# manyeyes/K2TransducerAsr

Hardware: AMD Instinct MI355X
Metric: RTFx (audio-sec/wall-sec) offline Zipformer greedy (higher is better)
Workload: dtype f32

## Files before the change

k2transducerasr_amd/csrc/attn.hip:

```cpp
#include "kernels.h"

namespace k2hip {

typedef float f32x16 __attribute__((ext_vector_type(16)));

namespace {

constexpr int PH = 4;
constexpr int R = 32;

template <int NG>
__global__ __launch_bounds__(512, 4) void k_attn_scores_softmax(const float* __restrict__ qkp, int ld,
                                                             const float* __restrict__ pp, float* __restrict__ aw, int B,
                                                             int T, int Tp, int H, int lds_stride, int koff0, int poff0) {
    constexpr int QH = 8 * NG;
    extern __shared__ __attribute__((aligned(16))) float S[];
    const int tid = threadIdx.x, lane = tid & 63, wave = tid >> 6;
    const int li = lane & 31, lh = lane >> 5;
    const int i0 = blockIdx.x * R, b = blockIdx.y, h = blockIdx.z;
    const float* base = qkp + (long long)b * T * ld;
    const int qoff = h * QH, koff = koff0 + h * QH, poff = poff0 + h * PH;
    const int ppld = H * PH;

    float4 fq[NG];
    {
        int row = i0 + li;
#pragma unroll
        for (int g = 0; g < NG; g++) {
            fq[g] = make_float4(0.f, 0.f, 0.f, 0.f);
            if (row < T) fq[g] = *reinterpret_cast<const float4*>(base + (long long)row * ld + qoff + 8 * g + 4 * lh);
        }
    }
    const int njt = (T + 31) / 32;
    float4 fkn[NG];
    auto load_keys = [&](int jt) {
        if (jt >= njt) return;
        const int j = min(jt * 32 + li, T - 1);
#pragma unroll
        for (int g = 0; g < NG; g++) fkn[g] = *reinterpret_cast<const float4*>(base + (long long)j * ld + koff + 8 * g + 4 * lh);
    };
    load_keys(wave);
    float4* PW = reinterpret_cast<float4*>(S + R * lds_stride);
    const int nlo = T - 1 - min(i0 + R - 1, T - 1), nwin = (2 * T - 2 - i0) - nlo + 1;
    for (int wdx = tid; wdx < nwin; wdx += 512) PW[wdx] = *reinterpret_cast<const float4*>(pp + (long long)(nlo + wdx) * ppld + h * PH);
    float4* PR = PW + (T + R);
    if (tid < R) PR[tid] = i0 + tid < T ? *reinterpret_cast<const float4*>(base + (long long)(i0 + tid) * ld + poff) : make_float4(0.f, 0.f, 0.f, 0.f);
    __syncthreads();

    for (int jt = wave; jt < njt; jt += 8) {
        int j = jt * 32 + li;
        float4 fk[NG];
#pragma unroll
        for (int g = 0; g < NG; g++) fk[g] = fkn[g];
        load_keys(jt + 8);
        f32x16 acc;
#pragma unroll
        for (int r = 0; r < 16; r++) acc[r] = 0.f;
#pragma unroll
        for (int g = 0; g < NG; g++) {
            acc = __builtin_amdgcn_mfma_f32_32x32x2f32(fq[g].x, fk[g].x, acc, 0, 0, 0);
            acc = __builtin_amdgcn_mfma_f32_32x32x2f32(fq[g].y, fk[g].y, acc, 0, 0, 0);
            acc = __builtin_amdgcn_mfma_f32_32x32x2f32(fq[g].z, fk[g].z, acc, 0, 0, 0);
            acc = __builtin_amdgcn_mfma_f32_32x32x2f32(fq[g].w, fk[g].w, acc, 0, 0, 0);
        }
        if (j < T) {
#pragma unroll
            for (int r0 = 0; r0 < 16; r0 += 8) {
                float4 e[8];
#pragma unroll
                for (int r = 0; r < 8; r++) {
                    const int rl = ((r0 + r) & 3) + 8 * ((r0 + r) >> 2) + 4 * lh;
                    e[r] = PW[T - 1 - min(i0 + rl, T - 1) + j - nlo];
                }
#pragma unroll
                for (int r = 0; r < 8; r++) {
                    const int rl = ((r0 + r) & 3) + 8 * ((r0 + r) >> 2) + 4 * lh;
                    const float4 pq = PR[rl];
                    S[rl * lds_stride + j] = acc[r0 + r] + (pq.x * e[r].x + pq.y * e[r].y + pq.z * e[r].z + pq.w * e[r].w);
                }
            }
        }
    }
    __syncthreads();

    float* out = aw + (((long long)h * B + b) * T) * Tp;
    if (Tp <= 1024) {
        float4 v[4][4];
        const int nk = (Tp + 255) >> 8;
#pragma unroll
        for (int rr = 0; rr < 4; rr++) {
            const float* srow = S + (wave * 4 + rr) * lds_stride;
#pragma unroll
            for (int k = 0; k < 4; k++) {
                const int j4 = lane * 4 + 256 * k;
                v[rr][k] = make_float4(-INFINITY, -INFINITY, -INFINITY, -INFINITY);
                if (k < nk && j4 < T) {
                    const float4 t = *reinterpret_cast<const float4*>(srow + j4);
                    v[rr][k].x = t.x;
                    if (j4 + 1 < T) v[rr][k].y = t.y;
                    if (j4 + 2 < T) v[rr][k].z = t.z;
                    if (j4 + 3 < T) v[rr][k].w = t.w;
                }
            }
        }
#pragma unroll
        for (int rr = 0; rr < 4; rr++) {
            const int i = i0 + wave * 4 + rr;
            if (i >= T) break;
            float mx = -INFINITY;
#pragma unroll
            for (int k = 0; k < 4; k++)
                if (k < nk) mx = fmaxf(fmaxf(fmaxf(mx, v[rr][k].x), fmaxf(v[rr][k].y, v[rr][k].z)), v[rr][k].w);
            mx = wave_max_dpp(mx);
            float sum = 0.f;
#pragma unroll
            for (int k = 0; k < 4; k++) {
                if (k >= nk) break;
                v[rr][k].x = __expf(v[rr][k].x - mx); v[rr][k].y = __expf(v[rr][k].y - mx);
                v[rr][k].z = __expf(v[rr][k].z - mx); v[rr][k].w = __expf(v[rr][k].w - mx);
                sum += (v[rr][k].x + v[rr][k].y) + (v[rr][k].z + v[rr][k].w);
            }
#pragma unroll
            for (int o = 32; o > 0; o >>= 1) sum += __shfl_xor(sum, o);
            const float inv = 1.0f / sum;
            float* orow = out + (long long)i * Tp;
#pragma unroll
            for (int k = 0; k < 4; k++) {
                const int j4 = lane * 4 + 256 * k;
                if (k < nk && j4 < Tp) *reinterpret_cast<float4*>(orow + j4) = make_float4(v[rr][k].x * inv, v[rr][k].y * inv, v[rr][k].z * inv, v[rr][k].w * inv);
            }
        }
        return;
    }
// ... 406 lines not shown
    }
    const int ct0 = blockIdx.z * tiles_per_z, ct1 = min(D >> 4, ct0 + tiles_per_z);
    const float* ar = cs_ + n * CS + 4 * kq;
    for (int ct = ct0 + wave; ct < ct1; ct += NWV) {
        const int col = ct * 16 + n;
        const float* wr = wout + (long long)col * Hc + 4 * kq;
        const float bvv = bias[col];
        float xr[4];
#pragma unroll
        for (int e = 0; e < 4; e++) {
            const int i = 4 * kq + e;
            xr[e] = i < T ? x[((long long)b * T + i) * D + col] : 0.f;
        }
        f32x4 acc0 = {0.f, 0.f, 0.f, 0.f}, acc1 = {0.f, 0.f, 0.f, 0.f};
        for (int c0 = 0; c0 < Hc; c0 += 64) {
            float4 w4[4], a4[4];
#pragma unroll
            for (int g = 0; g < 4; g++) {
                const bool ok = c0 + 16 * g + 4 * kq < Hc;
                w4[g] = ok ? *reinterpret_cast<const float4*>(wr + c0 + 16 * g) : make_float4(0.f, 0.f, 0.f, 0.f);
                a4[g] = ok ? *reinterpret_cast<const float4*>(ar + c0 + 16 * g) : make_float4(0.f, 0.f, 0.f, 0.f);
            }
#pragma unroll
            for (int g = 0; g < 4; g++) {
                if (g & 1) {
                    acc1 = __builtin_amdgcn_mfma_f32_16x16x4f32(a4[g].x, w4[g].x, acc1, 0, 0, 0);
                    acc1 = __builtin_amdgcn_mfma_f32_16x16x4f32(a4[g].y, w4[g].y, acc1, 0, 0, 0);
                    acc1 = __builtin_amdgcn_mfma_f32_16x16x4f32(a4[g].z, w4[g].z, acc1, 0, 0, 0);
                    acc1 = __builtin_amdgcn_mfma_f32_16x16x4f32(a4[g].w, w4[g].w, acc1, 0, 0, 0);
                } else {
                    acc0 = __builtin_amdgcn_mfma_f32_16x16x4f32(a4[g].x, w4[g].x, acc0, 0, 0, 0);
                    acc0 = __builtin_amdgcn_mfma_f32_16x16x4f32(a4[g].y, w4[g].y, acc0, 0, 0, 0);
                    acc0 = __builtin_amdgcn_mfma_f32_16x16x4f32(a4[g].z, w4[g].z, acc0, 0, 0, 0);
                    acc0 = __builtin_amdgcn_mfma_f32_16x16x4f32(a4[g].w, w4[g].w, acc0, 0, 0, 0);
                }
            }
        }
        float o[4];
#pragma unroll
        for (int e = 0; e < 4; e++) o[e] = acc0[e] + acc1[e] + bvv + xr[e];
        float* xp = x + ((long long)b * T + 4 * kq) * D + col;
#pragma unroll
        for (int e = 0; e < 4; e++)
            if (4 * kq + e < T) xp[(long long)e * D] = o[e];
    }
}

}

template <int NG>
static void attn_scores_launch(const Ctx& ctx, const float* qkp, int ld, const float* pp, float* aw, int B, int T, int Tp, int H, int koff0,
                               int poff0) {
    int lds_stride = Tp + 4;
    size_t lds = sizeof(float) * (R * lds_stride + 4 * (T + R) + 4 * R);
    const bool force_long = tunables().attn_long != 0;
    if (lds > 160 * 1024 || force_long) {
        hipLaunchKernelGGL(k_attn_scores_softmax_long<NG>, dim3(cdiv(T, R), B, H), dim3(256), 0, ctx.stream, qkp, ld, pp, aw, B, T, Tp, H, koff0,
                           poff0);
        K2_HIP(hipGetLastError());
        return;
    }
    static LdsAttrOnce lds_attr;
    lds_attr.ensure(k_attn_scores_softmax<NG>, 160 * 1024);
    dim3 grid(cdiv(T, R), B, H);
    hipLaunchKernelGGL(k_attn_scores_softmax<NG>, grid, dim3(512), lds, ctx.stream, qkp, ld, pp, aw, B, T, Tp, H, lds_stride, koff0, poff0);
    K2_HIP(hipGetLastError());
}

void attn_scores_softmax(const Ctx& ctx, const float* qkp, int ld, const float* pp, float* aw, int B, int T, int Tp, int H, int qh, int koff0,
                         int poff0) {
    K2_REQUIRE(Tp % 4 == 0 && Tp >= T, "attn: Tp=%d must be T=%d rounded up to 4", Tp, T);
    if (koff0 < 0) koff0 = H * qh;
    if (poff0 < 0) poff0 = 2 * H * qh;
    K2_REQUIRE(koff0 % 4 == 0 && poff0 % 4 == 0 && ld % 4 == 0, "attn: operand offsets must be multiples of 4 floats");
    ctx.add_flops(0.0, 2.0 * (qh + PH) * (double)T * T * B * H, 0);
    if (ctx.dry) return;
    switch (qh) {
        case 32: attn_scores_launch<4>(ctx, qkp, ld, pp, aw, B, T, Tp, H, koff0, poff0); break;
        case 24: attn_scores_launch<3>(ctx, qkp, ld, pp, aw, B, T, Tp, H, koff0, poff0); break;
        case 16: attn_scores_launch<2>(ctx, qkp, ld, pp, aw, B, T, Tp, H, koff0, poff0); break;
        default: failf(K2HIP_ERR_UNSUPPORTED, "attention head size %d unsupported (16, 24, 32)", qh);
    }
}

bool attn_av_out(const Ctx& ctx, const float* aw, const float* v, const float* wout, const float* bias, float* x, int B, int T, int KL, int Tp,
                 int H, int vh, int D) {
    const int HV = H * vh, Tk = (KL + 63) & ~63;
    const bool off = tunables().no_fused_av != 0;
    if (off || vh > 16 || HV % 4 != 0 || HV > 128 || D % 16 != 0 || Tp % 4 != 0 || Tp < KL) return false;
    ctx.add_flops(0.0, 2.0 * B * (double)T * HV * (KL + D), 0);
    if (ctx.dry) return true;
    const int strips = cdiv(T, 16) * B, ntile = D / 16;
    int cs = std::max(1, std::min(4, 512 / std::max(1, strips)));
    cs = std::min(cs, ntile);
    const int tiles_per_z = cdiv(ntile, cs);
    cs = cdiv(ntile, tiles_per_z);
    const size_t lds = sizeof(float) * 16 * (HV + 1);
    hipLaunchKernelGGL(k_attn_av_out<false>, dim3(cdiv(T, 16), B, cs), dim3(256), lds, ctx.stream, aw, v, wout, bias, x, B, T, KL, Tp, Tk, H, vh,
                       D, tiles_per_z, RingRef(), nullptr);
    K2_HIP(hipGetLastError());
    return true;
}

bool attn_av_out_ring(const Ctx& ctx, const float* aw, const RingRef& vals, const float* newrows, const float* wout, const float* bias, float* x,
                      int B, int T, int KL, int Tp, int H, int vh, int D) {
    const int HV = H * vh, Tk = (KL + 63) & ~63;
    K2_REQUIRE(vh <= 16 && HV % 4 == 0 && HV <= 128 && D % 16 == 0 && Tp % 4 == 0 && Tp >= KL && T <= 16,
// ... 71 lines not shown
```

k2transducerasr_amd/csrc/elementwise.hip:

```cpp
#include "kernels.h"

namespace k2hip {
namespace {

constexpr float kLogFloor = -23.025850929940457F;

__device__ __forceinline__ float fast_softplus(float z) { return z > 15.f ? z : __logf(1.0f + __expf(z)); }
__device__ __forceinline__ float swoosh_r(float v) { return fast_softplus(v - 1.0f) - 0.08f * v - 0.313261687f; }
__device__ __forceinline__ float fast_tanh(float v) {
    float e = __expf(-2.0f * fabsf(v));
    float t = (1.0f - e) / (1.0f + e);
    return v < 0.f ? -t : t;
}

__device__ __forceinline__ float sigm(float s) { return 1.0f / (1.0f + __expf(-s)); }
__device__ __forceinline__ float dswish(float v) { return v / (1.0f + __expf(1.0f - v)); }

inline int nblocks(long long n, int per) { return (int)((n + per - 1) / per); }

__global__ void k_pad_logfloor(const float* __restrict__ packed, const long long* __restrict__ off,
                               const long long* __restrict__ len, float* __restrict__ out, long long L) {
    int b = blockIdx.y;
    const float* src = packed + off[b];
    long long n = len[b];
    for (long long j = (long long)blockIdx.x * blockDim.x + threadIdx.x; j < L; j += (long long)gridDim.x * blockDim.x) {
        float v = j < n ? src[j] : 0.0f;
        out[(long long)b * L + j] = (v == 0.0f) ? kLogFloor : v;
    }
}
__global__ void k_pad_logfloor_dense(const float* __restrict__ feats, long long n, float* __restrict__ out, long long L) {
    int b = blockIdx.y;
    for (long long j = (long long)blockIdx.x * blockDim.x + threadIdx.x; j < L; j += (long long)gridDim.x * blockDim.x) {
        float v = j < n ? feats[(long long)b * n + j] : 0.0f;
        out[(long long)b * L + j] = (v == 0.0f) ? kLogFloor : v;
    }
}

template <int TPAD, bool DSWISH>
__global__ void k_conv0(const float* __restrict__ x, const float* __restrict__ w, const float* __restrict__ bias,
                        float* __restrict__ y, int B, int T, int F) {
    __shared__ float sw[72], sb[8];
    if (threadIdx.x < 72) sw[threadIdx.x] = w[threadIdx.x];
    if (threadIdx.x < 8) sb[threadIdx.x] = bias[threadIdx.x];
    __syncthreads();
    int T1 = T - 2 + 2 * TPAD;
    long long n = (long long)B * T1 * F;
    long long i = (long long)blockIdx.x * blockDim.x + threadIdx.x;
    if (i >= n) return;
    int f = (int)(i % F);
    long long bt = i / F;
    int t = (int)(bt % T1), b = (int)(bt / T1);
    float xin[3][3];
#pragma unroll
    for (int kt = 0; kt < 3; kt++)
#pragma unroll
        for (int kf = 0; kf < 3; kf++) {
            int ff = f + kf - 1, tt = t + kt - TPAD;
            xin[kt][kf] = (ff >= 0 && ff < F && tt >= 0 && tt < T) ? x[((long long)b * T + tt) * F + ff] : 0.f;
        }
    float o[8];
#pragma unroll
    for (int co = 0; co < 8; co++) {
        float s = sb[co];
#pragma unroll
        for (int kt = 0; kt < 3; kt++)
#pragma unroll
            for (int kf = 0; kf < 3; kf++) s += sw[(co * 3 + kt) * 3 + kf] * xin[kt][kf];
        o[co] = DSWISH ? dswish(s) : swoosh_r(s);
    }
    float4* yo = reinterpret_cast<float4*>(y + i * 8);
    yo[0] = make_float4(o[0], o[1], o[2], o[3]);
// ... 508 lines not shown
    const int q = (int)(i % W4);
    const long long bt = i / W4;
    const int t2 = (int)(bt % Td2), b = (int)(bt / Td2);
    float4 s = make_float4(0.f, 0.f, 0.f, 0.f);
    if (q < D4) {
        const float4 sc = reinterpret_cast<const float4*>(scale)[q];
        for (int k = 0; k < ds2; k++) {
            const int t = t2 * ds2 + k, tt = min(t, T - 1);
            const long long row = (long long)b * T + tt;
            const float4 o = q < Do4 ? reinterpret_cast<const float4*>(orig)[row * Do4 + q] : make_float4(0.f, 0.f, 0.f, 0.f);
            const float4 u = reinterpret_cast<const float4*>(xd)[((long long)b * Td + tt / ds) * D4 + q];
            const float4 v = make_float4(o.x + (u.x - o.x) * sc.x, o.y + (u.y - o.y) * sc.y, o.z + (u.z - o.z) * sc.z, o.w + (u.w - o.w) * sc.w);
            if (t < T) reinterpret_cast<float4*>(y)[row * D4 + q] = v;
            s.x += v.x * wgt[k]; s.y += v.y * wgt[k]; s.z += v.z * wgt[k]; s.w += v.w * wgt[k];
        }
    }
    if (q < D2_4) reinterpret_cast<float4*>(xd2)[((long long)b * Td2 + t2) * D2_4 + q] = s;
}
__global__ void k_convert_channels(const float* __restrict__ x, float* __restrict__ y, long long M, int Din4, int Dout4) {
    long long i = (long long)blockIdx.x * blockDim.x + threadIdx.x;
    if (i >= M * Dout4) return;
    long long m = i / Dout4;
    int q = (int)(i % Dout4);
    reinterpret_cast<float4*>(y)[i] = q < Din4 ? reinterpret_cast<const float4*>(x)[m * Din4 + q] : make_float4(0.f, 0.f, 0.f, 0.f);
}
__global__ void k_copy_cols(const float* __restrict__ x, int ldx, int xc, float* __restrict__ y, int ldy, int yc,
                            long long M, int n4) {
    long long i = (long long)blockIdx.x * blockDim.x + threadIdx.x;
    if (i >= M * n4) return;
    long long m = i / n4;
    int q = (int)(i % n4);
    *reinterpret_cast<float4*>(y + m * ldy + yc + 4 * q) = *reinterpret_cast<const float4*>(x + m * ldx + xc + 4 * q);
}

}

#define LAUNCH(kernel, grid, block, ...)                                        \
    do {                                                                        \
        if (!ctx.dry) {                                                         \
            hipLaunchKernelGGL(kernel, grid, block, 0, ctx.stream, __VA_ARGS__); \
            K2_HIP(hipGetLastError());                                          \
        }                                                                       \
    } while (0)

void pad_logfloor(const Ctx& ctx, const float* packed, const long long* d_off, const long long* d_len, float* out, int B,
                  long long L) {
    dim3 grid(std::min(nblocks(L, 256), 512), B);
    LAUNCH(k_pad_logfloor, grid, dim3(256), packed, d_off, d_len, out, L);
}
void pad_logfloor_dense(const Ctx& ctx, const float* feats, long long n_each, float* out, int B, long long L) {
    dim3 grid(std::min(nblocks(L, 256), 512), B);
    LAUNCH(k_pad_logfloor_dense, grid, dim3(256), feats, n_each, out, L);
}
void conv0_swoosh(const Ctx& ctx, const float* x, const float* w, const float* b, float* y, int B, int T, int F) {
    long long n = (long long)B * (T - 2) * F;
    LAUNCH((k_conv0<0, false>), dim3(nblocks(n, 256)), dim3(256), x, w, b, y, B, T, F);
}
void conv0_nopad_dswish(const Ctx& ctx, const float* x, const float* w, const float* b, float* y, int B, int T, int F) {
    long long n = (long long)B * (T - 2) * F;
    LAUNCH((k_conv0<0, true>), dim3(nblocks(n, 256)), dim3(256), x, w, b, y, B, T, F);
}
void conv0_pad1_dswish(const Ctx& ctx, const float* x, const float* w, const float* b, float* y, int B, int T, int F) {
    long long n = (long long)B * T * F;
    LAUNCH((k_conv0<1, true>), dim3(nblocks(n, 256)), dim3(256), x, w, b, y, B, T, F);
}
void basicnorm(const Ctx& ctx, const float* x, const float* log_eps, float* y, int M, int D) {
    K2_REQUIRE(D % 4 == 0 && D <= 1024, "basicnorm: D=%d unsupported", D);
    LAUNCH(k_basicnorm, dim3(nblocks(M, 4)), dim3(256), x, log_eps, y, M, D);
}
void dwconv7x7(const Ctx& ctx, const float* x, const float* w_kc, const float* b, float* y, int B, int Tin, int T, int tpad,
               int F, int C) {
    ctx.add_flops(0.0, 2.0 * B * T * (double)F * C * 49, 0);
    if (C % DW7_CG == 0 && F <= 24 && !tunables().dw7_tiled && T >= 48 && (long long)F * C * 4 < (1ll << 31)) {
        if (ctx.dry) return;
        const int TR = T >= 256 ? 64 : 32;
        size_t lds = sizeof(float) * ((size_t)DW7_RING * (F + 6) * 32 + 49 * 32);
        static LdsAttrOnce lds_attr;
        lds_attr.ensure(k_dwconv7x7_slide, 96 * 1024);
        hipLaunchKernelGGL(k_dwconv7x7_slide, dim3(C / DW7_CG, cdiv(T, TR), B), dim3(192), lds, ctx.stream, x, w_kc, b, y, Tin, T, tpad, F,
                           C, TR);
        K2_HIP(hipGetLastError());
        return;
    }
    if (C % DW7_CG == 0 && F <= 24) {
        if (ctx.dry) return;
        size_t lds = sizeof(float) * ((size_t)(DW7_TT + 6) * (F + 6) * 32 + 49 * 32);
        hipLaunchKernelGGL(k_dwconv7x7_tiled, dim3(C / DW7_CG, cdiv(T, DW7_TT), B), dim3(192), lds, ctx.stream, x, w_kc, b, y, Tin, T,
                           tpad, F, C);
        K2_HIP(hipGetLastError());
        return;
    }
    long long n = (long long)B * T * F * (C / 4);
    LAUNCH(k_dwconv7x7, dim3(nblocks(n, 256)), dim3(256), x, w_kc, b, y, B, Tin, T, tpad, F, C);
}
void biasnorm(const Ctx& ctx, const float* x, const float* bias, const float* log_scale, float* y, int M, int D) {
    K2_REQUIRE(D % 4 == 0 && D <= 1024, "biasnorm: D=%d unsupported", D);
    LAUNCH((k_biasnorm<false>), dim3(nblocks(M, 4)), dim3(256), x, nullptr, bias, log_scale, nullptr, y, M, D);
}
void biasnorm_bypass(const Ctx& ctx, const float* x, const float* orig, const float* nbias, const float* log_scale,
                     const float* scale, float* y, int M, int D) {
    K2_REQUIRE(D % 4 == 0 && D <= 1024, "biasnorm: D=%d unsupported", D);
    LAUNCH((k_biasnorm<true>), dim3(nblocks(M, 4)), dim3(256), x, orig, nbias, log_scale, scale, y, M, D);
}
void biasnorm_bypass_downsample(const Ctx& ctx, const float* x, const float* orig, const float* nbias, const float* log_scale, const float* scale,
                                float* y, const float* bias2, float* xd2, int B, int T, int D, int ds2, int D2) {
    K2_REQUIRE(D % 4 == 0 && D <= 1024 && D2 % 4 == 0 && D2 <= 1024 && ds2 >= 1 && ds2 <= 16, "biasnorm + downsample: D=%d D2=%d ds=%d unsupported", D, D2, ds2);
// ... 92 lines not shown
```

k2transducerasr_amd/csrc/engine.cpp:

```cpp
#include <cstring>
#include <thread>

#include "engine.h"
#include "lattice_ref.h"
#include "ctc_lattice_ref.h"

#include <climits>
#include <cmath>

namespace k2hip {

namespace {
constexpr int kTailFrames = 19;
}

Engine::Engine(const std::string& weights, const char* overrides, int device) : device_(device) {
    tunables_init_from_env();
    model_.reset(new Model(weights, overrides));
    int n = 0;
    if (hipGetDeviceCount(&n) != hipSuccess || n <= 0)
        failf(K2HIP_ERR_NO_DEVICE, "no HIP device visible: libk2hip has no CPU fallback");
    if (device < 0 || device >= n) failf(K2HIP_ERR_NO_DEVICE, "device %d out of range (have %d)", device, n);
    K2_HIP(hipSetDevice(device));
    model_->upload(device);
// ... 2004 lines not shown
            } else {
                fill.assign((size_t)n_ids + 1, std::min(3, model_->cfg().V - 1));
                ids = fill.data();
            }
            const AlignPlan p = align_plan(B, Tp, nf, ids, lens, max_tokens);
            K2_REQUIRE(dev[k_stay] && dev[k_emit] && buf_bytes[k_stay] >= 4 * p.plane_floats && buf_bytes[k_emit] >= 4 * p.plane_floats,
                       "debug_op_run %s: the planes need %lld floats each", op, p.plane_floats);
            if (cells) K2_REQUIRE(dev[k_enc] && buf_bytes[k_enc] >= 4 * (int64_t)B * Tp * model_->cfg().J, "debug_op_run %s: enc is too short", op);
            else
                K2_REQUIRE(dev[k_ts] && dev[k_lp] && dev[k_sc] && buf_bytes[k_ts] >= 4 * (int64_t)B * max_tokens &&
                               buf_bytes[k_lp] >= 4 * (int64_t)B * max_tokens && buf_bytes[k_sc] >= 8 * (int64_t)B,
                           "debug_op_run %s: the result buffers are too short", op);
            SearchOut out;
            SearchExtras ex;
            run_sized([&](const Ctx& cc) {
                out = SearchOut(*cc.arena, B, cells ? 1 : max_tokens);
                ex = align_device(cc, cells ? static_cast<const float*>(dev[k_enc]) : nullptr, Tp, p, out, static_cast<float*>(dev[k_stay]),
                                  static_cast<float*>(dev[k_emit]), cells, !cells);
            });
            K2_HIP(hipStreamSynchronize(stream_));
            if (!cells) {
                K2_HIP(copy_blocking(dev[k_ts], out.timestamps(), 4 * (size_t)B * max_tokens, hipMemcpyDeviceToDevice));
                K2_HIP(copy_blocking(dev[k_lp], ex.align_lp, 4 * (size_t)B * max_tokens, hipMemcpyDeviceToDevice));
                K2_HIP(copy_blocking(dev[k_sc], ex.align_scores, 8 * (size_t)B, hipMemcpyDeviceToDevice));
            }
        } else if (name == "ctc_lattice") {
            K2_REQUIRE(n_bufs == 9, "debug_op_run %s: %d buffers", op, n_bufs);
            for (int k = 0; k < n_bufs; k++) P();
            const int R = I(), Tp = I(), H = I(), max_tokens = I();
            K2_REQUIRE(R > 0 && Tp > 0 && H > 0 && max_tokens > 0, "debug_op_run %s: bad shape", op);
            K2_REQUIRE(bufs[4] && buf_bytes[4] >= 4 * (int64_t)H && (!bufs[1] || buf_bytes[1] >= 4 * (int64_t)R) && (!bufs[2] || buf_bytes[2] >= 4 * (int64_t)H),
                       "debug_op_run %s: lens / n_frames / stream_of are too short", op);
            const int32_t* lens = static_cast<const int32_t*>(bufs[4]);
            int64_t n_ids = 0;
            for (int h = 0; h < H; h++) n_ids += std::max(lens[h], 0);
            K2_REQUIRE(n_ids == 0 || (bufs[3] && buf_bytes[3] >= 8 * n_ids), "debug_op_run %s: ids are too short", op);
            const CtcAlignPlan p = ctc_align_plan(R, Tp, static_cast<const int32_t*>(bufs[1]), H, static_cast<const int32_t*>(bufs[2]),
                                                  static_cast<const int64_t*>(bufs[3]), lens, max_tokens);
            K2_REQUIRE(dev[0] && buf_bytes[0] >= 4 * (int64_t)R * Tp * model_->cfg().V, "debug_op_run %s: log_probs is too short", op);
            K2_REQUIRE(dev[5] && dev[6] && dev[7] && dev[8] && buf_bytes[5] >= 4 * (int64_t)H * max_tokens && buf_bytes[6] >= 4 * (int64_t)H * max_tokens &&
                           buf_bytes[7] >= 4 * (int64_t)H * max_tokens && buf_bytes[8] >= 8 * (int64_t)H,
                       "debug_op_run %s: the result buffers are too short", op);
            SearchOut out;
            SearchExtras ex;
            run_sized([&](const Ctx& cc) {
                out = SearchOut(*cc.arena, H, max_tokens);
                ex = ctc_align_device(cc, static_cast<const float*>(dev[0]), R, Tp, p, out);
            });
            K2_HIP(hipStreamSynchronize(stream_));
            K2_HIP(copy_blocking(dev[5], out.timestamps(), 4 * (size_t)H * max_tokens, hipMemcpyDeviceToDevice));
            K2_HIP(copy_blocking(dev[6], ex.align_end, 4 * (size_t)H * max_tokens, hipMemcpyDeviceToDevice));
            K2_HIP(copy_blocking(dev[7], ex.align_lp, 4 * (size_t)H * max_tokens, hipMemcpyDeviceToDevice));
            K2_HIP(copy_blocking(dev[8], ex.align_scores, 8 * (size_t)H, hipMemcpyDeviceToDevice));
        } else if (name == "basicnorm") {
            float *x = P(), *le = P(), *y = P();
            const int M = I(), D = I();
            basicnorm(c, x, le, y, M, D);
        } else if (name == "conv0_pad1_dswish" || name == "conv0_nopad_dswish") {
            float *x = P(), *w = P(), *b = P(), *y = P();
            const int B = I(), T = I(), Fq = I();
            if (name == "conv0_pad1_dswish") conv0_pad1_dswish(c, x, w, b, y, B, T, Fq);
            else conv0_nopad_dswish(c, x, w, b, y, B, T, Fq);
        } else {
            failf(K2HIP_ERR_INVALID, "debug_op_run: unknown op '%s'", op);
        }
    } catch (const Error& e) {
        if (e.code == K2HIP_ERR_INVALID && strncmp(e.what(), "debug_op_run", 12) != 0) throw Error(K2HIP_ERR_UNSUPPORTED, e.what());
        throw;
    }
    if (!took) failf(K2HIP_ERR_UNSUPPORTED, "debug_op_run %s: the launcher does not take this shape", op);
    K2_REQUIRE(ni == n_iargs && nbuf == n_bufs, "debug_op_run %s: %d int arguments and %d buffers passed, %d and %d used", op, n_iargs, n_bufs, ni,
               nbuf);
    K2_HIP(hipStreamSynchronize(stream_));
    std::vector<unsigned char> g((size_t)kGuard);
    for (int k = 0; k < n_bufs; k++) {
        if (!dev[k]) continue;
        const char* p = static_cast<const char*>(dev[k]);
        for (int side = 0; side < 2; side++) {
            K2_HIP(copy_blocking(g.data(), side ? p + buf_bytes[k] : p - kGuard, (size_t)kGuard, hipMemcpyDeviceToHost));
            for (int64_t i = 0; i < kGuard; i++)
                if (g[(size_t)i] != 0xff)
                    failf(K2HIP_ERR_INVALID, "debug_op_run %s: buffer %d written %s its end (guard byte %lld)", op, k, side ? "past" : "before",
                          (long long)(side ? i : kGuard - i));
        }
    }
    for (int k = 0; k < n_bufs; k++)
        if (dev[k] && (out_mask >> k & 1u)) K2_HIP(copy_blocking(bufs[k], dev[k], (size_t)buf_bytes[k], hipMemcpyDeviceToHost));
}

void Engine::debug_gemm_trace(int M, int N, int K, int act, bool with_res, int cfg, unsigned long long* out, int64_t cap, int* n_wg, int* n_waves) {
    K2_HIP(hipSetDevice(device_));
    GemmForceGuard force(cfg);
    GemmArgs g;
    g.lda = K; g.ldw = K; g.ldc = N; g.M = M; g.N = N; g.K = K; g.act = act; g.ldr = N;
    const GemmPlan p = plan_gemm(g, gemm_force());
    K2_REQUIRE(p.family == GemmFamily::DMA || p.family == GemmFamily::RING || p.family == GemmFamily::PIPE,
               "trace: LDS-DMA (0, 5, 7, 9, 10, 11), ring (100+) and pipelined (2000+) configurations only");
    *n_wg = cdiv(M, p.BM) * cdiv(N, p.BN);
    *n_waves = p.waves;
    const int64_t words = (int64_t)*n_wg * p.waves * 64;
    K2_REQUIRE(words <= cap, "trace buffer too small: need %lld words", (long long)words);
    std::vector<float> h((size_t)std::max((int64_t)M * K, std::max((int64_t)N * K, (int64_t)M * N)));
    uint32_t s = 12345u;
    for (auto& v : h) { s = s * 1664525u + 1013904223u; v = ((s >> 8) * (1.0f / 8388608.0f)) - 1.0f; }
    DevBufs dev;
    float* A = dev.alloc<float>((size_t)M * K);
// ... 54 lines not shown
```

k2transducerasr_amd/csrc/gemm.hip:

```cpp
#include <algorithm>
#include <cmath>
#include <cstdlib>
#include <map>
#include <mutex>
#include <type_traits>

#include "kernels.h"

#pragma clang diagnostic ignored "-Winline-asm"

namespace k2hip {

typedef float f32x16 __attribute__((ext_vector_type(16)));
typedef float f32x4 __attribute__((ext_vector_type(4)));

namespace {


__device__ __forceinline__ float fast_softplus(float z) {
    return z > 15.f ? z : __logf(1.0f + __expf(z));
}
__device__ __forceinline__ float apply_act(float v, int act) {
    switch (act) {
        case ACT_SWOOSH_L: return fast_softplus(v - 4.0f) - 0.08f * v - 0.035f;
        case ACT_SWOOSH_R: return fast_softplus(v - 1.0f) - 0.08f * v - 0.313261687f;
        case ACT_TANH: {
            float e = __expf(-2.0f * fabsf(v));
            float t = (1.0f - e) / (1.0f + e);
            return v < 0.f ? -t : t;
        }
        case ACT_SIGMOID: return 1.0f / (1.0f + __expf(-v));
        case ACT_RELU: return fmaxf(v, 0.f);
        case ACT_DOUBLE_SWISH: return v / (1.0f + __expf(1.0f - v));
        default: return v;
    }
}

__device__ __forceinline__ float4 sel4(bool ok, float4 v) {
    return make_float4(ok ? v.x : 0.f, ok ? v.y : 0.f, ok ? v.z : 0.f, ok ? v.w : 0.f);
}

struct Rows32 {
    static __device__ __forceinline__ int off(int r) { return (r & 3) + 8 * (r >> 2); }
};
struct Rows16 {
    static __device__ __forceinline__ int off(int e) { return e; }
};
template <int NV, typename ROWS>
__device__ __forceinline__ void epilogue_rows(const GemmArgs& g, float (&v)[NV], int row0, int col, float* __restrict__ C,
                                              const float* __restrict__ R, const float (&rres)[NV], bool use_rres,
                                              const float* __restrict__ mulp, const float* __restrict__ biasp, bool bias_loaded = false,
                                              float bias_value = 0.f) {
    if (col >= g.N) return;
    const float bv = bias_loaded ? bias_value : (biasp ? biasp[col] : 0.f);
    const bool act_on = g.act_cols == 0 || col < g.act_cols;
    float rv[NV], mv[NV], ov[NV];
    float bs = 0.f;
    const bool has_res = R != nullptr || use_rres;
    if (use_rres) {
#pragma unroll
        for (int n = 0; n < NV; n++) rv[n] = rres[n];
    } else if (R) {
#pragma unroll
        for (int n = 0; n < NV; n++) {
            const int row = min(row0 + ROWS::off(n), g.M - 1);
            rv[n] = R[(long long)(g.res_div > 1 ? row / g.res_div : row) * g.ldr + col];
        }
    }
    if (mulp) {
#pragma unroll
        for (int n = 0; n < NV; n++) mv[n] = mulp[(long long)min(row0 + ROWS::off(n), g.M - 1) * g.ldm + col];
    }
    if (g.byp_orig) {
        bs = g.byp_scale[col];
#pragma unroll
        for (int n = 0; n < NV; n++) ov[n] = g.byp_orig[(long long)min(row0 + ROWS::off(n), g.M - 1) * g.ld_orig + col];
    }
#pragma unroll
// ... 893 lines not shown
    const int Tc = 1 << lgTc, CH = 1 << lgCH, lgQ = lgTc - (TPT == 1 ? 0 : TPT == 2 ? 1 : TPT == 4 ? 2 : 3), Q = 1 << lgQ;
    for (int w = tid; w < (S << (lgCH + lgQ)); w += nthreads) {
        const int ch = w & (CH - 1), sq = w >> lgCH, q = sq & (Q - 1), s = sq >> lgQ;
        if (b0 + s >= Bn) continue;
        const int c = c0 + ch, tq = q * TPT;
        const float* cp = colL + ((s << lgCH) + ch) * CL + tq;
        float col[TPT + Kc - 1], wc[Kc];
#pragma unroll
        for (int j = 0; j < TPT + Kc - 1; j++) col[j] = cp[j];
#pragma unroll
        for (int k = 0; k < Kc; k++) wc[k] = wcl[ch * KcP + k];
        float le[TPT], re[TPT], bcv, bwv;
        if (use_pre) {
            bcv = pre.bcv;
            bwv = pre.bwv;
#pragma unroll
            for (int i = 0; i < TPT; i++) {
                le[i] = pre.le[i < PRE::TPT0 ? i : 0];
                re[i] = pre.re[i < PRE::TPT0 ? i : 0];
            }
        } else {
            bcv = g.cf_bc[c];
            bwv = g.cf_bw[c];
#pragma unroll
            for (int i = 0; i < TPT; i++) {
                const int t = tq + i, il = min(t, K - 1), ir = min(max(t - (Tc - K), 0), K - 1);
                const float lv = g.cf_sc[(long long)c * K + il], rv = g.cf_sc[(long long)D * K + (long long)c * K + ir];
                le[i] = t < K ? lv : 0.f;
                re[i] = t >= Tc - K ? rv : 0.f;
            }
        }
        float* yp = g.C + ((long long)m0 + (s << lgTc) + tq) * g.ldc + c;
        float xw[TPT];
#pragma unroll
        for (int i = 0; i < TPT; i++) xw[i] = bwv;
        {
            const float* xcol = colL + ((s << lgCH) + ch) * CL + pad;
            const float* wrow = wwl + ch * K + pad - tq;
            for (int tt = 0; tt < Tc; tt++) {
                const float xv = xcol[tt];
#pragma unroll
                for (int i = 0; i < TPT; i++) {
                    const int k = tt - i + pad - tq;
                    if (k >= 0 && k < K) xw[i] += wrow[tt - i] * xv;
                }
            }
        }
#pragma unroll
        for (int i = 0; i < TPT; i++) {
            float xc = bcv;
#pragma unroll
            for (int k = 0; k < Kc; k++) xc += wc[k] * col[i + k];
            const float z = xw[i] * (1.0f + (le[i] + re[i])) + xc;
            yp[(long long)i * g.ldc] = fast_softplus(z - 1.0f) - 0.08f * z - 0.313261687f;
        }
    }
}

template <int BM, int BN, int NV, int NTHR>
__device__ __forceinline__ void conv_tail(const GemmArgs& g, const ConvPre<BM, BN, NTHR>& pre, const float (&fin)[NV], float* smem, int m0, int n0, int wc,
                                          int lrow0, int li, int tid) {
    constexpr int CH = BN / 2, lgCH = CH == 16 ? 4 : 5, TPT0 = ConvPre<BM, BN, NTHR>::TPT0;
    const int Tc = g.cf_Tc, lgTc = pre.lgTc, K = g.cf_K, pad = pre.pad, Kc = pre.Kc, CL = pad + Tc, S = BM >> lgTc, KcP = Kc | 1;
    const int Bn = g.M >> lgTc, b0 = m0 >> lgTc, c0 = n0 >> 1, D = g.N >> 1;
    float* colL = smem;
    float* wcl = colL + S * CH * CL;
    float* wwl = wcl + CH * KcP;
    __syncthreads();
    {
        const int ch = wc * 16 + (li & 15);
#pragma unroll
        for (int n = 0; n < NV; n++) {
            const float v = fin[n] + pre.bias;
            const float other = __shfl_xor(v, 16, 64);
            const float gated = v * (1.0f / (1.0f + __expf(-other)));
            const int lrow = lrow0 + Rows32::off(n);
            const int s = lrow >> lgTc, t = lrow & (Tc - 1);
            if ((li & 16) == 0) colL[(s * CH + ch) * CL + pad + t] = gated;
        }
    }
    const int npc = pre.npc, TPS = 1 << pre.lgTPS, cs = pre.cs, cr = pre.cr;
    const bool live = pre.live;
    const float inv_pad = 1.0f / (float)pad;
    const int nper = (npc + TPS - 1) >> pre.lgTPS;
#pragma unroll
    for (int u = 0; u < 8; u++) {
        const int rem = cr + u * TPS;
        if (u < nper && live && rem < npc) {
            const int ch = __float2int_rz(((float)rem + 0.5f) * inv_pad), r = rem - ch * pad;
            colL[(cs * CH + ch) * CL + r] = pre.cv[u];
        }
    }
    {
        const int lgKc = 31 - __builtin_clz(Kc);
#pragma unroll
        for (int u = 0; u < 4; u++) {
            const int idx = tid + u * NTHR;
            if (idx < CH * Kc) wcl[(idx >> lgKc) * KcP + (idx & (Kc - 1))] = pre.wv[u];
            if (idx < CH * K) wwl[idx] = pre.uv[u];
        }
    }
    __syncthreads();
#define K2_CONV_OUT(KT_, TPT_, PRE_) conv_outputs<KT_, TPT_>(g, pre, PRE_, colL, wcl, wwl, CL, KcP, lgTc, lgCH, S, Bn, b0, c0, m0, D, tid, NTHR)
    if (pre.full) {
        switch (K) {
            case 31: K2_CONV_OUT(31, TPT0, true); break;
            case 15: K2_CONV_OUT(15, TPT0, true); break;
// ... 506 lines not shown
```

k2transducerasr_amd/csrc/kernels.h:

```cpp
#pragma once
#include "common.h"

namespace k2hip {

#ifdef K2HIP_DEV
#define K2HIP_DEV_SWITCH(name, def) int name = def
#else
#define K2HIP_DEV_SWITCH(name, def) static constexpr int name = def
#endif
struct Tunables {
    int no_glu_epilogue = 0;
    int attn_long = 0;
    int no_fused_av = 0;
    int fused_vproj_min_t = 4;
    int no_fused_vproj = 0;
    int no_fused_conv = 0;
    int conformer_gemm_scores = 0;
    int dw7_tiled = 0;
    int dw1d_tt = 0;
    int lstm_seq = 0;
    int greedy_one_part = 0;
    int greedy_parts = 0;
    int beam_launches = 0;
    int beam_parts = 0;
// ... 127 lines not shown
struct GemmPlan {
    GemmFamily family = GemmFamily::REG;
    int idx = 0;
    int mode = MODE_PLAIN;
    int ablate = 0;
    int BM = 0, BN = 0, waves = 0;
};
struct GemmForce {
    enum Kind { AUTO, CFG, RING, PIPE, P16 } kind = AUTO;
    int idx = -1;
    int ablate = 0;
    bool dma = true;
};
GemmForce decode_gemm_force(int code);
GemmPlan plan_gemm(const GemmArgs& a, const GemmForce& f);
int gemm_kind(const GemmArgs& a, const GemmPlan& p);
int glu_conv_ring_entry(int B, int Tc, int D, int K);
void debug_force_gemm_cfg(int code);
GemmForce gemm_force();
struct GemmForceGuard {
    explicit GemmForceGuard(int code) { debug_force_gemm_cfg(code); }
    ~GemmForceGuard() { debug_force_gemm_cfg(-1); }
    GemmForceGuard(const GemmForceGuard&) = delete;
    GemmForceGuard& operator=(const GemmForceGuard&) = delete;
};
void linear(const Ctx& ctx, const float* A, int lda, const float* W, const float* bias, float* C, int ldc, int M, int K,
            int N, int act = ACT_NONE, const float* res = nullptr, int ldr = 0);

struct RingRef {
    float* pool = nullptr;
    long long slot_stride = 0;
    long long off = 0;
    const int* slots = nullptr;
    const int* chunks = nullptr;
};

void attn_scores_softmax(const Ctx& ctx, const float* qkp, int ld, const float* pp, float* aw, int B, int T, int Tp, int H, int qh = 32,
                         int koff0 = -1, int poff0 = -1);

bool attn_av_out(const Ctx& ctx, const float* aw, const float* v, const float* wout, const float* bias, float* x, int B, int T, int KL, int Tp,
                 int H, int vh, int D);
bool attn_av_out_ring(const Ctx& ctx, const float* aw, const RingRef& vals, const float* newrows, const float* wout, const float* bias, float* x,
                      int B, int T, int KL, int Tp, int H, int vh, int D);
void attn_proj_av_out_ring(const Ctx& ctx, const float* aw, const RingRef& vals, const float* xin, const float* win, const float* bin,
                           const float* wout, const float* bias, float* xout, int B, int T, int KL, int Tp, int H, int vh, int D);

void nonlin_av_out_ring(const Ctx& ctx, const float* aw, const RingRef& cache, const float* hid, int ldh, const float* wout, const float* bias,
                        float* x, int B, int T, int KL, int Tp, int Hc, int D);

void pad_logfloor(const Ctx& ctx, const float* packed, const long long* d_off, const long long* d_len, float* out, int B,
                  long long L);
void pad_logfloor_dense(const Ctx& ctx, const float* feats, long long n_each, float* out, int B, long long L);
void conv0_swoosh(const Ctx& ctx, const float* x, const float* w, const float* b, float* y, int B, int T, int F);
void conv0_pad1_dswish(const Ctx& ctx, const float* x, const float* w, const float* b, float* y, int B, int T, int F);
void dwconv7x7(const Ctx& ctx, const float* x, const float* w_kc, const float* b, float* y, int B, int Tin, int Tout, int tpad,
               int F, int C);
void biasnorm(const Ctx& ctx, const float* x, const float* bias, const float* log_scale, float* y, int M, int D);
void biasnorm_bypass(const Ctx& ctx, const float* x, const float* orig, const float* nbias, const float* log_scale,
                     const float* scale, float* y, int M, int D);
void biasnorm_bypass_downsample(const Ctx& ctx, const float* x, const float* orig, const float* nbias, const float* log_scale, const float* scale,
                                float* y, const float* bias2, float* xd2, int B, int T, int D, int ds2, int D2);
struct LayerTail {
    const float* bias2 = nullptr;
    float* xd2 = nullptr;
    int ds2 = 1, D2 = 0;
};
void bypass(const Ctx& ctx, const float* orig, const float* x, const float* scale, float* y, int M, int D);
void glu_sigmoid(const Ctx& ctx, const float* x, float* y, int M, int D);
void tanh_gate(const Ctx& ctx, const float* x, float* y, int M, int Hc);
void mul_cols(const Ctx& ctx, float* a, const float* x, int ldx, int col0, int M, int N);
void dwconv1d_swoosh(const Ctx& ctx, const float* x, const float* w_kd, const float* b, float* y, int B, int T, int D, int K);
void glu_dwconv1d_swoosh(const Ctx& ctx, const float* x2, const float* w_kd, const float* b, float* y, int B, int T, int D,
                          int K);
void glu_dwconv1d_dswish(const Ctx& ctx, const float* x2, const float* w_kd, const float* b, float* y, int B, int T, int D,
                          int K);
void conv0_nopad_dswish(const Ctx& ctx, const float* x, const float* w, const float* b, float* y, int B, int T, int F);
void lstm_cell(const Ctx& ctx, const float* gx, long long ldgx, const float* gh, int ldgh, float* c, float* hf, int B, int Hh);
void add_inplace(const Ctx& ctx, float* a, const float* b, long long n);
void lstm_cell_rows(const Ctx& ctx, const float* gates, float* c, float* hf, int rows, int Hh);
void lstm_add_frame(const Ctx& ctx, const float* Y, long long SY, const float* hp, long long pstride, int S, float* h, float* x1, int n, int B,
                    int T, int D, int lo, int s);
void lstm_norm_frame(const Ctx& ctx, const float* x1, const float* fp, long long pstride, int S, const float* b2_0, const float* eps0,
                     long long lstride, float* Y, long long SY, int n, int B, int T, int D, int lo, int s);
void gather_rows(const Ctx& ctx, const float* pool, long long slot_stride, long long off, const int* slots, float* out, int B, int width);
void scatter_rows(const Ctx& ctx, float* pool, long long slot_stride, long long off, const int* slots, const float* in, int ldin, int B, int width);
void basicnorm(const Ctx& ctx, const float* x, const float* log_eps, float* y, int M, int D);
void conformer_qprep(const Ctx& ctx, const float* qkv, const float* bias_u, const float* bias_v, float* qu, float* qv, int M,
                     int D, float scaling, int ldq = 0 );
void conformer_softmax_shift_stream(const Ctx& ctx, float* ac, const float* bd, const long long* plen, int B, int H, int Tc, int left,
                                    int KLp, int NPp);
void slice_rows(const Ctx& ctx, const float* in, float* out, int B, int Tin, int row0, int Tout, int D);
void dwconv_valid_dswish(const Ctx& ctx, const float* cat, const float* w_kd, const float* bias, float* y, int B, int Tc, int D, int K);
void conformer_softmax_shift(const Ctx& ctx, float* ac, const float* bd, int Z, int T, int Tp, int NPp);
bool conformer_scores_softmax(const Ctx& ctx, const float* qu, const float* qv, const float* kmat, int ldk, const float* pp, float* aw, int B, int H,
                              int T, int Tp, int D, int ldq = 0, const float* bias_u = nullptr, const float* bias_v = nullptr, float scaling = 1.0f);
void downsample(const Ctx& ctx, const float* x, const float* bias, float* y, int B, int T, int D, int ds, int Din = 0);
void upsample_combine(const Ctx& ctx, const float* orig, const float* xd, const float* scale, float* y, int B, int T,
                      int Td, int D, int ds, int Dorig = 0);
void upsample_combine_downsample(const Ctx& ctx, const float* orig, const float* xd, const float* scale, float* y, const float* bias2,
                                 float* xd2, int B, int T, int Td, int D, int ds, int Dorig, int D2, int ds2);
void convert_channels(const Ctx& ctx, const float* x, float* y, int M, int Din, int Dout);
struct FullDimSegs {
    const float* src[8];
    int ld[8], col1[8], n = 0;
    const float* lz_orig = nullptr;
    const float* lz_xd = nullptr;
// ... 284 lines not shown
```

k2transducerasr_amd/csrc/online.hip:

```cpp
#include "kernels.h"

namespace k2hip {
namespace {

__device__ __forceinline__ float fast_softplus(float z) { return z > 15.f ? z : __logf(1.0f + __expf(z)); }
__device__ __forceinline__ float swoosh_r(float v) { return fast_softplus(v - 1.0f) - 0.08f * v - 0.313261687f; }
__device__ __forceinline__ float sigm(float s) { return 1.0f / (1.0f + __expf(-s)); }

__global__ void k_convnext_cat(const float* __restrict__ a3, float* __restrict__ pool, long long slot_stride,
                               long long embed_off, const int* __restrict__ slots, float* __restrict__ cat, float* __restrict__ byp, int B,
                               int T3, int Tc, int F, int C) {
    long long n = (long long)B * (T3 + 3) * F * C;
    long long i = (long long)blockIdx.x * blockDim.x + threadIdx.x;
    if (i >= n) return;
    int c = (int)(i % C);
    long long p = i / C;
    int f = (int)(p % F);
    long long bt = p / F;
    int t = (int)(bt % (T3 + 3)), b = (int)(bt / (T3 + 3));
    float v;
    if (t < 3) {
        float* cp = pool + (long long)slots[b] * slot_stride + embed_off + ((long long)c * 3 + t) * F + f;
        v = *cp;
        *cp = a3[(((long long)b * T3 + (Tc - 3 + t)) * F + f) * C + c];
    } else {
        v = a3[(((long long)b * T3 + (t - 3)) * F + f) * C + c];
        if (t - 3 < Tc) byp[(((long long)b * Tc + (t - 3)) * F + f) * C + c] = v;
    }
    cat[i] = v;
}

template <bool GATE>
__global__ void k_cat_shift(float* __restrict__ pool, long long slot_stride, long long off, const int* __restrict__ slots,
                            const float* __restrict__ newrows, int ldn, float* __restrict__ cat, int B, int L, int Tc, int width) {
    auto newrow = [&](const float* p) {
        float4 v = *reinterpret_cast<const float4*>(GATE ? p + width : p);
        if (GATE) {
            const float4 sg = *reinterpret_cast<const float4*>(p);
            v = make_float4(v.x * tanhf(sg.x), v.y * tanhf(sg.y), v.z * tanhf(sg.z), v.w * tanhf(sg.w));
        }
        return v;
    };
    const int w4 = width >> 2;
    const long long n = (long long)B * Tc * w4;
    const long long i = (long long)blockIdx.x * blockDim.x + threadIdx.x;
    if (i >= n) return;
    const int c = (int)(i % w4) * 4;
    const long long br = i / w4;
    const int r0 = (int)(br % Tc), b = (int)(br / Tc);
    float* cache = pool + (long long)slots[b] * slot_stride + off + c;
    const float* nw = newrows + (long long)b * Tc * ldn + c;
    float* ct = cat + (long long)b * (L + Tc) * width + c;
    const float4 mine = newrow(nw + (long long)r0 * ldn);
    *reinterpret_cast<float4*>(ct + (long long)(L + r0) * width) = mine;
    if (r0 >= L) return;
    float4 cur = *reinterpret_cast<const float4*>(cache + (long long)r0 * width);
    for (int rb = r0; rb < L; rb += 8 * Tc) {
        float4 nx[8];
#pragma unroll
// ... 441 lines not shown
```

Before: 23590.

## Compute positional attention scores with MFMA and use a leaner softplus

The positional term of the attention scores used to be a per-element 4-wide dot product over an LDS window. It is now computed with 32x32x2 MFMA tiles and written diagonally into the score buffer. The content-score MFMA then starts its accumulator from those values instead of adding the dot product afterwards, which frees the LDS that held the window. Separately, the Swoosh activations share a new softplus that calls the raw hardware log2 plus a compensated multiply by ln2 instead of __logf, and a debug op is added to compare it against the old form.

After: 23870, median of 6. 1.2% higher.

```diff
diff --git a/k2transducerasr_amd/csrc/act.h b/k2transducerasr_amd/csrc/act.h
--- /dev/null
+++ b/k2transducerasr_amd/csrc/act.h
@@ -0,0 +1,21 @@
+#pragma once
+#include <hip/hip_runtime.h>
+
+namespace k2hip {
+
+__device__ __forceinline__ float softplus_libm(float z) { return z > 15.f ? z : __logf(1.0f + __expf(z)); }
+
+__device__ __forceinline__ float softplus_ge1(float z) {
+    const float y = __builtin_amdgcn_logf(1.0f + __expf(z));
+    const float c = __builtin_bit_cast(float, 0x3f317217u), c_lo = __builtin_bit_cast(float, 0x3377d1cfu);
+    const float t = c * y;
+    float e = __builtin_fmaf(y, c, -t);
+    e = __builtin_fmaf(y, c_lo, e);
+    const float r = __builtin_fmaf(c, y, e);
+    return z > 15.f ? z : r;
+}
+
+__device__ __forceinline__ float swoosh_l(float v) { return softplus_ge1(v - 4.0f) - 0.08f * v - 0.035f; }
+__device__ __forceinline__ float swoosh_r(float v) { return softplus_ge1(v - 1.0f) - 0.08f * v - 0.313261687f; }
+
+}
diff --git a/k2transducerasr_amd/csrc/attn.hip b/k2transducerasr_amd/csrc/attn.hip
--- a/k2transducerasr_amd/csrc/attn.hip
+++ b/k2transducerasr_amd/csrc/attn.hip
@@ -40,11 +40,42 @@
         for (int g = 0; g < NG; g++) fkn[g] = *reinterpret_cast<const float4*>(base + (long long)j * ld + koff + 8 * g + 4 * lh);
     };
     load_keys(wave);
-    float4* PW = reinterpret_cast<float4*>(S + R * lds_stride);
-    const int nlo = T - 1 - min(i0 + R - 1, T - 1), nwin = (2 * T - 2 - i0) - nlo + 1;
-    for (int wdx = tid; wdx < nwin; wdx += 512) PW[wdx] = *reinterpret_cast<const float4*>(pp + (long long)(nlo + wdx) * ppld + h * PH);
-    float4* PR = PW + (T + R);
-    if (tid < R) PR[tid] = i0 + tid < T ? *reinterpret_cast<const float4*>(base + (long long)(i0 + tid) * ld + poff) : make_float4(0.f, 0.f, 0.f, 0.f);
+
+    {
+        const int nlo = T - 1 - min(i0 + R - 1, T - 1), nwin = (2 * T - 2 - i0) - nlo + 1;
+        float2 fp = make_float2(0.f, 0.f);
+        if (i0 + li < T) fp = *reinterpret_cast<const float2*>(base + (long long)(i0 + li) * ld + poff + 2 * lh);
+        const float* pw = pp + h * PH + 2 * lh;
+        auto load_window = [&](int t) {
+            return *reinterpret_cast<const float2*>(pw + (long long)min(nlo + t * 32 + li, 2 * T - 2) * ppld);
+        };
+        float2 fw = load_window(wave);
+        for (int t = wave; t * 32 < nwin; t += 8) {
+            const float2 fwn = load_window(t + 8);
+            f32x16 acc;
+#pragma unroll
+            for (int r = 0; r < 16; r++) acc[r] = 0.f;
+            acc = __builtin_amdgcn_mfma_f32_32x32x2f32(fp.x, fw.x, acc, 0, 0, 0);
+            acc = __builtin_amdgcn_mfma_f32_32x32x2f32(fp.y, fw.y, acc, 0, 0, 0);
+            fw = fwn;
+            const int j00 = nlo + t * 32 + i0 - (T - 1);
+            const int j0 = j00 + li + 4 * lh;
+            float* sp = S + 4 * lh * lds_stride + j0;
+            if (j00 >= 0 && j00 + 62 < T) {
+#pragma unroll
+                for (int r = 0; r < 16; r++) {
+                    const int ro = (r & 3) + 8 * (r >> 2);
+                    sp[ro * lds_stride + ro] = acc[r];
+                }
+            } else {
+#pragma unroll
+                for (int r = 0; r < 16; r++) {
+                    const int ro = (r & 3) + 8 * (r >> 2);
+                    if ((unsigned)(j0 + ro) < (unsigned)T) sp[ro * lds_stride + ro] = acc[r];
+                }
+            }
+        }
+    }
     __syncthreads();
 
     for (int jt = wave; jt < njt; jt += 8) {
@@ -53,9 +84,10 @@
 #pragma unroll
         for (int g = 0; g < NG; g++) fk[g] = fkn[g];
         load_keys(jt + 8);
+        float* sp = S + 4 * lh * lds_stride + min(j, T - 1);
         f32x16 acc;
 #pragma unroll
-        for (int r = 0; r < 16; r++) acc[r] = 0.f;
+        for (int r = 0; r < 16; r++) acc[r] = sp[((r & 3) + 8 * (r >> 2)) * lds_stride];
 #pragma unroll
         for (int g = 0; g < NG; g++) {
             acc = __builtin_amdgcn_mfma_f32_32x32x2f32(fq[g].x, fk[g].x, acc, 0, 0, 0);
@@ -65,20 +97,7 @@
         }
         if (j < T) {
 #pragma unroll
-            for (int r0 = 0; r0 < 16; r0 += 8) {
-                float4 e[8];
-#pragma unroll
-                for (int r = 0; r < 8; r++) {
-                    const int rl = ((r0 + r) & 3) + 8 * ((r0 + r) >> 2) + 4 * lh;
-                    e[r] = PW[T - 1 - min(i0 + rl, T - 1) + j - nlo];
-                }
-#pragma unroll
-                for (int r = 0; r < 8; r++) {
-                    const int rl = ((r0 + r) & 3) + 8 * ((r0 + r) >> 2) + 4 * lh;
-                    const float4 pq = PR[rl];
-                    S[rl * lds_stride + j] = acc[r0 + r] + (pq.x * e[r].x + pq.y * e[r].y + pq.z * e[r].z + pq.w * e[r].w);
-                }
-            }
+            for (int r = 0; r < 16; r++) sp[((r & 3) + 8 * (r >> 2)) * lds_stride] = acc[r];
         }
     }
     __syncthreads();
@@ -591,7 +610,7 @@
 static void attn_scores_launch(const Ctx& ctx, const float* qkp, int ld, const float* pp, float* aw, int B, int T, int Tp, int H, int koff0,
                                int poff0) {
     int lds_stride = Tp + 4;
-    size_t lds = sizeof(float) * (R * lds_stride + 4 * (T + R) + 4 * R);
+    size_t lds = sizeof(float) * R * lds_stride;
     const bool force_long = tunables().attn_long != 0;
     if (lds > 160 * 1024 || force_long) {
         hipLaunchKernelGGL(k_attn_scores_softmax_long<NG>, dim3(cdiv(T, R), B, H), dim3(256), 0, ctx.stream, qkp, ld, pp, aw, B, T, Tp, H, koff0,
diff --git a/k2transducerasr_amd/csrc/elementwise.hip b/k2transducerasr_amd/csrc/elementwise.hip
--- a/k2transducerasr_amd/csrc/elementwise.hip
+++ b/k2transducerasr_amd/csrc/elementwise.hip
@@ -1,3 +1,4 @@
+#include "act.h"
 #include "kernels.h"
 
 namespace k2hip {
@@ -5,8 +6,6 @@
 
 constexpr float kLogFloor = -23.025850929940457F;
 
-__device__ __forceinline__ float fast_softplus(float z) { return z > 15.f ? z : __logf(1.0f + __expf(z)); }
-__device__ __forceinline__ float swoosh_r(float v) { return fast_softplus(v - 1.0f) - 0.08f * v - 0.313261687f; }
 __device__ __forceinline__ float fast_tanh(float v) {
     float e = __expf(-2.0f * fabsf(v));
     float t = (1.0f - e) / (1.0f + e);
@@ -17,6 +16,14 @@
 __device__ __forceinline__ float dswish(float v) { return v / (1.0f + __expf(1.0f - v)); }
 
 inline int nblocks(long long n, int per) { return (int)((n + per - 1) / per); }
+
+__global__ void k_act_forms(const float* __restrict__ x, float* __restrict__ y_lean, float* __restrict__ y_libm, int act, long long n) {
+    for (long long i = (long long)blockIdx.x * blockDim.x + threadIdx.x; i < n; i += (long long)gridDim.x * blockDim.x) {
+        const float v = x[i];
+        y_lean[i] = act == ACT_SWOOSH_L ? swoosh_l(v) : swoosh_r(v);
+        y_libm[i] = act == ACT_SWOOSH_L ? softplus_libm(v - 4.0f) - 0.08f * v - 0.035f : softplus_libm(v - 1.0f) - 0.08f * v - 0.313261687f;
+    }
+}
 
 __global__ void k_pad_logfloor(const float* __restrict__ packed, const long long* __restrict__ off,
                                const long long* __restrict__ len, float* __restrict__ out, long long L) {
@@ -631,6 +638,11 @@
     dim3 grid(std::min(nblocks(L, 256), 512), B);
     LAUNCH(k_pad_logfloor_dense, grid, dim3(256), feats, n_each, out, L);
 }
+void act_forms(const Ctx& ctx, const float* x, float* y_lean, float* y_libm, int act, long long n) {
+    K2_REQUIRE(act == ACT_SWOOSH_L || act == ACT_SWOOSH_R, "act_forms: act %d is neither SwooshL (1) nor SwooshR (2)", act);
+    if (n <= 0) return;
+    LAUNCH(k_act_forms, dim3(std::min(nblocks(n, 256), 4096)), dim3(256), x, y_lean, y_libm, act, n);
+}
 void conv0_swoosh(const Ctx& ctx, const float* x, const float* w, const float* b, float* y, int B, int T, int F) {
     long long n = (long long)B * (T - 2) * F;
     LAUNCH((k_conv0<0, false>), dim3(nblocks(n, 256)), dim3(256), x, w, b, y, B, T, F);
diff --git a/k2transducerasr_amd/csrc/engine.cpp b/k2transducerasr_amd/csrc/engine.cpp
--- a/k2transducerasr_amd/csrc/engine.cpp
+++ b/k2transducerasr_amd/csrc/engine.cpp
@@ -2080,6 +2080,13 @@
             K2_HIP(copy_blocking(dev[6], ex.align_end, 4 * (size_t)H * max_tokens, hipMemcpyDeviceToDevice));
             K2_HIP(copy_blocking(dev[7], ex.align_lp, 4 * (size_t)H * max_tokens, hipMemcpyDeviceToDevice));
             K2_HIP(copy_blocking(dev[8], ex.align_scores, 8 * (size_t)H, hipMemcpyDeviceToDevice));
+        } else if (name == "act_forms") {
+            const int act = I();
+            const long long n = L();
+            float *x = P(), *y_lean = P(), *y_libm = P();
+            K2_REQUIRE(n >= 0 && x && y_lean && y_libm && buf_bytes[0] >= 4 * n && buf_bytes[1] >= 4 * n && buf_bytes[2] >= 4 * n,
+                       "debug_op_run act_forms: three buffers of n = %lld floats are needed", n);
+            act_forms(c, x, y_lean, y_libm, act, n);
         } else if (name == "basicnorm") {
             float *x = P(), *le = P(), *y = P();
             const int M = I(), D = I();
diff --git a/k2transducerasr_amd/csrc/gemm.hip b/k2transducerasr_amd/csrc/gemm.hip
--- a/k2transducerasr_amd/csrc/gemm.hip
+++ b/k2transducerasr_amd/csrc/gemm.hip
@@ -5,6 +5,7 @@
 #include <mutex>
 #include <type_traits>
 
+#include "act.h"
 #include "kernels.h"
 
 #pragma clang diagnostic ignored "-Winline-asm"
@@ -17,13 +18,10 @@
 namespace {
 
 
-__device__ __forceinline__ float fast_softplus(float z) {
-    return z > 15.f ? z : __logf(1.0f + __expf(z));
-}
 __device__ __forceinline__ float apply_act(float v, int act) {
     switch (act) {
-        case ACT_SWOOSH_L: return fast_softplus(v - 4.0f) - 0.08f * v - 0.035f;
-        case ACT_SWOOSH_R: return fast_softplus(v - 1.0f) - 0.08f * v - 0.313261687f;
+        case ACT_SWOOSH_L: return swoosh_l(v);
+        case ACT_SWOOSH_R: return swoosh_r(v);
         case ACT_TANH: {
             float e = __expf(-2.0f * fabsf(v));
             float t = (1.0f - e) / (1.0f + e);
@@ -1023,7 +1021,7 @@
 #pragma unroll
             for (int k = 0; k < Kc; k++) xc += wc[k] * col[i + k];
             const float z = xw[i] * (1.0f + (le[i] + re[i])) + xc;
-            yp[(long long)i * g.ldc] = fast_softplus(z - 1.0f) - 0.08f * z - 0.313261687f;
+            yp[(long long)i * g.ldc] = swoosh_r(z);
         }
     }
 }
diff --git a/k2transducerasr_amd/csrc/kernels.h b/k2transducerasr_amd/csrc/kernels.h
--- a/k2transducerasr_amd/csrc/kernels.h
+++ b/k2transducerasr_amd/csrc/kernels.h
@@ -203,6 +203,7 @@
                   long long L);
 void pad_logfloor_dense(const Ctx& ctx, const float* feats, long long n_each, float* out, int B, long long L);
 void conv0_swoosh(const Ctx& ctx, const float* x, const float* w, const float* b, float* y, int B, int T, int F);
+void act_forms(const Ctx& ctx, const float* x, float* y_lean, float* y_libm, int act, long long n);
 void conv0_pad1_dswish(const Ctx& ctx, const float* x, const float* w, const float* b, float* y, int B, int T, int F);
 void dwconv7x7(const Ctx& ctx, const float* x, const float* w_kc, const float* b, float* y, int B, int Tin, int Tout, int tpad,
                int F, int C);
diff --git a/k2transducerasr_amd/csrc/online.hip b/k2transducerasr_amd/csrc/online.hip
--- a/k2transducerasr_amd/csrc/online.hip
+++ b/k2transducerasr_amd/csrc/online.hip
@@ -1,10 +1,9 @@
+#include "act.h"
 #include "kernels.h"
 
 namespace k2hip {
 namespace {
 
-__device__ __forceinline__ float fast_softplus(float z) { return z > 15.f ? z : __logf(1.0f + __expf(z)); }
-__device__ __forceinline__ float swoosh_r(float v) { return fast_softplus(v - 1.0f) - 0.08f * v - 0.313261687f; }
 __device__ __forceinline__ float sigm(float s) { return 1.0f / (1.0f + __expf(-s)); }
 
 __global__ void k_convnext_cat(const float* __restrict__ a3, float* __restrict__ pool, long long slot_stride,
```
